# mdolab/dafoam

Hardware: AMD Instinct MI355X
Metric: adjoint_gmres_iterations_per_sec (higher is better)
Workload: dtype f64

## Files before the change

dafoam_amd/_capi.py:

```python
from __future__ import annotations

import ctypes as C
import os

import numpy as np

from .meshgen import FoamCase

_HERE = os.path.dirname(os.path.abspath(__file__))
LIB_PATH = os.environ.get("DAFOAM_AMD_LIB") or os.path.join(_HERE, "lib", "libdafoam_amd.so")

SOLVER_IDS = {"DASimpleFoam": 0, "DAScalarTransportFoam": 1, "DARhoSimpleFoam": 2, "DATurboFoam": 3}
PATCH_TYPES = {"patch": 0, "wall": 1, "symmetry": 2, "cyclic": 3}

c_double_p = C.POINTER(C.c_double)
c_int_p = C.POINTER(C.c_int)
c_ll_p = C.POINTER(C.c_longlong)


class das_case_t(C.Structure):
    _fields_ = [
        ("solver", C.c_int),
        ("n_points", C.c_int),
        ("n_faces", C.c_int),
# ... 238 lines not shown
    "das_set_dense_eig_callback": (C.c_int, [_VP]),
    "das_debug_gmres_dr_host": (C.c_int, [C.c_longlong, _VP, _VP, _VP, c_double_p, c_double_p, C.c_int, C.c_int, C.c_double, C.c_double, C.c_longlong, c_double_p, C.c_int,
                                          c_double_p, c_double_p]),
    "das_debug_gmres_dr_restart": (C.c_int, [C.c_int, C.c_int, c_double_p, c_double_p, c_double_p, c_double_p, c_double_p]),
    "das_ksp_get_status": (C.c_int, [_VP, c_int_p, c_int_p, c_int_p, c_int_p]),
    "das_ksp_get_pc_stability": (C.c_int, [_VP, C.POINTER(C.c_double), c_int_p]),
    "das_ksp_get_pc_subdomains": (C.c_int, [_VP, c_int_p, c_double_p]),
    "das_ksp_get_pc_node_out": (C.c_int, [_VP, c_int_p]),
    "das_mesh_metrics": (C.c_int, [C.c_int, c_double_p, C.c_int, C.c_int, C.c_int, c_int_p, c_int_p, c_int_p, c_int_p, c_double_p, c_double_p, c_double_p, c_double_p, c_double_p]),
    "das_ksp_get_coarse": (C.c_int, [_VP, c_int_p]),
    "das_ksp_coarse_sparse_az_active": (C.c_int, [_VP]),
    "das_ksp_set_global_coarse": (C.c_int, [_VP, _VP, C.c_int, C.c_int, c_int_p]),
    "das_ksp_run_fixed_device": (C.c_int, [_VP, _VP, _VP, _VP, C.c_int]),
    "das_ksp_begin_device": (C.c_int, [_VP, _VP, _VP, _VP, C.c_int]),
    "das_ksp_advance": (C.c_int, [_VP, _VP, C.c_int]),
    "das_ksp_end": (C.c_int, [_VP, _VP]),
    "das_ksp_destroy": (None, [_VP]),
    "das_set_owned_mask": (C.c_int, [_VP, C.POINTER(C.c_ubyte)]),
    "das_comm_load_rccl": (C.c_int, []),
    "das_comm_unique_id": (C.c_int, [C.c_char_p]),
    "das_comm_init_rccl": (C.c_int, [_VP, C.c_int, C.c_int, C.c_char_p]),
    "das_comm_set_halo": (C.c_int, [_VP, C.c_int, c_int_p, c_ll_p, c_int_p, c_ll_p, c_int_p, C.c_longlong, c_int_p]),
    "das_set_exchange_cb": (C.c_int, [_VP, _VP, _VP]),
    "das_set_pc_overlap": (C.c_int, [_VP, C.POINTER(C.c_ubyte), C.c_int, c_ll_p, c_int_p, c_ll_p, c_int_p]),
    "das_set_gather_cb": (C.c_int, [_VP, _VP, _VP]),
    "das_comm_is_native": (C.c_int, [_VP]),
    "das_comm_reset": (C.c_int, [_VP]),
    "das_set_comm": (C.c_int, [_VP, _VP, _VP, _VP]),
    "das_set_stream": (C.c_int, [_VP, _VP]),
    "das_get_elapsed_clock_time": (C.c_double, [_VP]),
    "das_get_elapsed_cpu_time": (C.c_double, [_VP]),
    "das_timer_avg_ms": (C.c_double, [_VP, C.c_char_p]),
    "das_debug_orth_bench": (C.c_int, [C.c_longlong, C.c_int, C.c_int, C.c_int, C.c_int, C.c_int, C.POINTER(C.c_double), C.POINTER(C.c_double)]),
    "das_debug_krylov_dots2": (C.c_int, [C.c_longlong, C.c_int, C.c_int, _VP, C.c_longlong, c_double_p, c_double_p]),
    "das_debug_krylov_dcgs2_update": (C.c_int, [C.c_longlong, C.c_int, C.c_int, _VP, C.c_longlong, C.c_int, c_double_p, C.c_double, C.c_double, c_double_p]),
    "das_debug_krylov_multidot": (C.c_int, [C.c_longlong, C.c_int, C.c_int, _VP, C.c_longlong, c_double_p, c_double_p]),
    "das_debug_krylov_multiaxpy": (C.c_int, [C.c_longlong, C.c_int, C.c_int, _VP, C.c_longlong, c_double_p, C.c_int, _VP, C.c_longlong]),
    "das_debug_krylov_lincomb": (C.c_int, [C.c_longlong, C.c_int, C.c_int, _VP, C.c_longlong, c_double_p, c_double_p, C.c_longlong]),
    "das_debug_krylov_scale_to": (C.c_int, [C.c_longlong, C.c_double, C.c_int, _VP, _VP, C.c_longlong]),
    "das_debug_krylov_block_tn": (C.c_int, [C.c_longlong, C.c_int, C.c_int, c_double_p, C.c_longlong, C.c_longlong, c_double_p, C.c_longlong, c_double_p]),
    "das_debug_krylov_block_nn_sub": (C.c_int, [C.c_longlong, C.c_int, C.c_int, c_double_p, C.c_longlong, c_double_p, c_double_p, C.c_longlong]),
    "das_debug_krylov_block_right_mult": (C.c_int, [C.c_longlong, C.c_int, c_double_p, C.c_longlong, c_double_p]),
    "das_debug_krylov_block_lincomb": (C.c_int, [C.c_longlong, C.c_int, C.c_int, c_double_p, C.c_longlong, c_double_p, c_double_p, C.c_longlong]),
    "das_debug_krylov_block_spmm": (C.c_int, [C.c_longlong, C.c_int, c_ll_p, c_int_p, c_double_p, c_double_p, C.c_longlong, c_double_p, C.c_longlong]),
    "das_timer_count": (C.c_longlong, [_VP, C.c_char_p]),
    "das_timer_reset": (None, [_VP]),
    "das_timer_enable": (None, [_VP, C.c_int]),
}

_lib = None


def declared_symbols():
    return sorted(_SIGS)


def lib():
    global _lib
    if _lib is None:
        if not os.path.exists(LIB_PATH):
            raise ImportError(
                f"{LIB_PATH} not found: build the HIP extension first (python -c 'import __graft_entry__ as g; g.build()'). "
                "dafoam_amd has no CPU fallback."
            )
        L = C.CDLL(LIB_PATH)
        for name, (res, args) in _SIGS.items():
# ... 45 lines not shown
```

dafoam_amd/csrc/das_device.hip:

```cpp
#include <algorithm>
#include <cmath>
#include <ctime>
#include <functional>
#include <numeric>
#include <thread>

#include "das_case.hpp"
#include "das_jaccon.hpp"
#include "das_bilu.hpp"
#include "das_comm.hpp"
#include "das_block.hpp"
#include "das_color.hpp"
#include "das_opmat.hpp"
#include "das_graph.hpp"
#include "das_volcoord.hpp"
#include "das_cellfn.hpp"
#include "das_simple.hpp"

#include <omp.h>

namespace das {

template <class T, bool RHO, class G = double>
__global__ __launch_bounds__(256) void k_grad(DevMeshT<G> m, ResParams prm, const T* __restrict__ W, T* nut, T* gU, T* gP, T* gN, T* gH) {
// ... 506 lines not shown
#pragma unroll
        for (int t = 0; t < UNROLL; t++)
#pragma unroll
            for (int r = 0; r < RPT; r++) q[t][r] = (double)V[(long long)(i + t) * ldv + kk[r]];
        if (Vlo) {
#pragma unroll
            for (int t = 0; t < UNROLL; t++)
#pragma unroll
                for (int r = 0; r < RPT; r++) q[t][r] += (double)Vlo[(long long)(i + t) * ldv + kk[r]];
        }
#pragma unroll
        for (int t = 0; t < UNROLL; t++)
#pragma unroll
            for (int r = 0; r < RPT; r++) { as[r] += s[i + t] * q[t][r]; ac[r] += c[i + t] * q[t][r]; }
    }
    for (; i < j; i++)
#pragma unroll
        for (int r = 0; r < RPT; r++) {
            const double q = (double)V[(long long)i * ldv + kk[r]] + (Vlo ? (double)Vlo[(long long)i * ldv + kk[r]] : 0.0);
            as[r] += s[i] * q; ac[r] += c[i] * q;
        }
#pragma unroll
    for (int r = 0; r < RPT; r++) {
        const long long k = k0 + (long long)r * blockDim.x;
        if (k >= n) continue;
        const double u = (double)V[(long long)j * ldv + k] + (Vlo ? (double)Vlo[(long long)j * ldv + k] : 0.0);
        const double qj = (u - as[r]) * ralpha, un = (v[k] - gamma * u - ac[r]) * ralpha;
        const VT qh = (VT)qj, uh = (VT)un;
        V[(long long)j * ldv + k] = qh;
        V[(long long)(j + 1) * ldv + k] = uh;
        if (Vlo) { Vlo[(long long)j * ldv + k] = (float)(qj - (double)qh); Vlo[(long long)(j + 1) * ldv + k] = (float)(un - (double)uh); }
    }
}
template <class VT>
__global__ __launch_bounds__(256) void k_lincomb(long long n, int m, const VT* __restrict__ V, long long ldv, const double* __restrict__ c,
                                                 double* __restrict__ y, const float* __restrict__ Vlo = nullptr) {
    long long k = (long long)blockIdx.x * blockDim.x + threadIdx.x;
    if (k >= n) return;
    double s = 0.0;
    if (Vlo) for (int i = 0; i < m; i++) s += c[i] * ((double)V[(long long)i * ldv + k] + (double)Vlo[(long long)i * ldv + k]);
    else for (int i = 0; i < m; i++) s += c[i] * (double)V[(long long)i * ldv + k];
    y[k] = s;
}
template <class TI, class TO>
__global__ void k_scale_to(long long n, double a, const TI* __restrict__ x, TO* __restrict__ y, const float* __restrict__ xlo = nullptr,
                           float* __restrict__ ylo = nullptr) {
    long long k = (long long)blockIdx.x * blockDim.x + threadIdx.x;
    if (k >= n) return;
    const double val = a * ((double)x[k] + (xlo ? (double)xlo[k] : 0.0));
    const TO yh = (TO)val;
    y[k] = yh;
    if (ylo) ylo[k] = (float)(val - (double)yh);
}
static inline size_t multidot_partial_size(long long n, int m) { return (size_t)(m + 1) * nblk(n, MD_CHUNK); }
template <class VT>
static void launch_multidot(hipStream_t st, long long n, int m, const VT* V, long long ldv, const double* w, double* partial, double* out) {
    const int nb = nblk(n, MD_CHUNK);
    hipLaunchKernelGGL(k_multidot, dim3(nb), dim3(256), 0, st, n, m, V, ldv, w, partial, nb);
    hipLaunchKernelGGL(k_reduce, dim3(m + 1), dim3(256), 0, st, nb, (const double*)partial, out);
}
template <int ROWS>
static inline long long multidot2_nbw(long long n) { return 4LL * nblk(n, 256 * ROWS); }
static inline size_t multidot2_partial_size(long long n, int K) { return (size_t)2 * K * (size_t)multidot2_nbw<MD2_ROWS>(n); }
template <int ROWS, class VT>
static void launch_multidot2_pass(hipStream_t st, long long n, int K, const VT* V, long long ldv, const VT* u, const double* v, double* partial) {
    hipLaunchKernelGGL((k_multidot2<ROWS, VT, VT>), dim3(nblk(n, 256 * ROWS)), dim3(256), 0, st, n, K, V, ldv, u, v, partial, multidot2_nbw<ROWS>(n));
}
template <class VT>
static void launch_multidot2(hipStream_t st, long long n, int K, const VT* V, long long ldv, const VT* u, const double* v, double* partial, double* out) {
    launch_multidot2_pass<MD2_ROWS, VT>(st, n, K, V, ldv, u, v, partial);
    hipLaunchKernelGGL(k_reduce, dim3(2 * K), dim3(256), 0, st, (int)multidot2_nbw<MD2_ROWS>(n), (const double*)partial, out);
}
template <int UNROLL, int RPT, class VT>
static void launch_dcgs2_update(hipStream_t st, long long n, int j, VT* V, long long ldv, const double* sc, double gamma, double ralpha, const double* v,
                                float* Vlo) {
    hipLaunchKernelGGL((k_dcgs2_update<UNROLL, RPT, VT>), dim3(nblk(n, 256 * RPT)), dim3(256), 0, st, n, j, V, ldv, sc, gamma, ralpha, v, Vlo);
}
template <class VT, class WT>
static void launch_multiaxpy(hipStream_t st, long long n, int m, const VT* V, long long ldv, const double* h, WT* w, const float* Vlo) {
    hipLaunchKernelGGL(k_multiaxpy, dim3(nblk(n, 256)), dim3(256), 0, st, n, m, V, ldv, h, w, Vlo);
}
template <class VT>
static void launch_lincomb(hipStream_t st, long long n, int m, const VT* V, long long ldv, const double* c, double* y, const float* Vlo) {
    hipLaunchKernelGGL(k_lincomb, dim3(nblk(n, 256)), dim3(256), 0, st, n, m, V, ldv, c, y, Vlo);
}
template <class TI, class TO>
static void launch_scale_to(hipStream_t st, long long n, double a, const TI* x, TO* y, const float* xlo, float* ylo) {
    hipLaunchKernelGGL(k_scale_to, dim3(nblk(n, 256)), dim3(256), 0, st, n, a, x, y, xlo, ylo);
}
static constexpr int TSG_CHUNKS = 1024;
static inline int tsgemm_kpad(int K) { return (K + 16 * TSG_TILES - 1) / (16 * TSG_TILES) * (16 * TSG_TILES); }
static inline size_t tsgemm_partial_size(int K) { return (size_t)TSG_CHUNKS * tsgemm_kpad(K) * 16; }
static void launch_tsgemm_tn(hipStream_t st, long long n, int K, int sv, const double* V, long long ldv, const double* W, long long ldw, double* partial,
                             double* C) {
    long long rpc = (n + TSG_CHUNKS - 1) / TSG_CHUNKS;
    rpc = (rpc + 15) / 16 * 16;
    const int Kpad = tsgemm_kpad(K);
    const int gy = Kpad / (16 * TSG_TILES);
    DAS_CHECK((((ldv | ldw) & 1) != 0) || ((((uintptr_t)V | (uintptr_t)W) & 15) == 0), DAS_ERR_ARG,
              "block V^T W: even leading dimensions need 16-byte aligned blocks");
    hipLaunchKernelGGL(k_tsgemm_tn, dim3(TSG_CHUNKS / TSG_WAVES, gy), dim3(64 * TSG_WAVES), 0, st, n, K, sv, V, ldv, W, ldw, rpc, Kpad, partial);
    hipLaunchKernelGGL(k_tsgemm_reduce, dim3(nblk((long long)K * sv, 4)), dim3(256), 0, st, K, sv, Kpad, (long long)TSG_CHUNKS, (const double*)partial, C);
}
static void launch_tsgemm_nn_sub(hipStream_t st, long long n, int K, int sv, const double* V, long long ldv, const double* C, double* W, long long ldw) {
    hipLaunchKernelGGL(k_tsgemm_nn_sub, dim3(nblk(n, 256)), dim3(256), 0, st, n, K, sv, V, ldv, C, W, ldw);
}
static void launch_block_right_mult(hipStream_t st, long long n, int sv, double* W, long long ldw, const double* T) {
    hipLaunchKernelGGL(k_block_right_mult, dim3(nblk(n, 256)), dim3(256), 0, st, n, sv, W, ldw, T);
// ... 1646 lines not shown
}

static void pc_apply(das_solver* s, das_ksp* k, const double* b, double* x) {
    hipEvent_t ev = nullptr;
    s->timer.begin("pc", s->stream, ev);
    if (k->useBilu) {
        if (k->rasOverlap) {
            DAS_HIP(hipMemcpyAsync(k->pcin.p, b, (size_t)s->n * sizeof(double), hipMemcpyDeviceToDevice, s->stream));
            s->halo.gather_overlap(k->pcin.p, s->stream);
            bilu_apply(k->bilu, k->pcin.p, x, s->stream);
            s->halo.zero_overlap(x, s->stream);
        } else {
            bilu_apply(k->bilu, b, x, s->stream);
        }
        s->timer.end("pc", s->stream, ev);
        return;
    }
    const int mlv = k->pc.maxLevels;
    const size_t lvlBytes = (size_t)((mlv + 2 * PC_PF + 4) >> 1) * sizeof(double);
    if (k->pc.useLDS)
        hipLaunchKernelGGL(k_ras_apply<true>, dim3(k->pc.nBlocks), dim3(PC_THREADS), lvlBytes + (size_t)k->pc.maxLocal * sizeof(double), s->stream,
                           k->pc.view, b, x, mlv);
    else
        hipLaunchKernelGGL(k_ras_apply<false>, dim3(k->pc.nBlocks), dim3(PC_THREADS), lvlBytes, s->stream, k->pc.view, b, x, mlv);
    s->timer.end("pc", s->stream, ev);
}

static void gmres_ws(das_solver* s, das_ksp* k) {
    const long long n = s->n;
    long long restart = std::min<long long>(s->opt.geti("adjEqnOption.gmresRestart"), s->opt.geti("adjEqnOption.gmresMaxIters"));
    long long budget = (long long)(32.0 * 1024 * 1024 * 1024);
    auto it = s->opt.i.find("amd.maxKrylovBytes");
    if (it != s->opt.i.end()) budget = it->second;
    const long long maxVec = std::max<long long>(3, budget / (8 * n));
    restart = std::max<long long>(1, std::min<long long>(restart, maxVec - 2));
    long long wantVec = std::max<long long>(restart + 2, std::min<long long>(maxVec, 1002));
    if ((size_t)wantVec * (size_t)n * sizeof(double) < ((size_t)4 << 30) || getenv("DAS_NO_VMM")) wantVec = restart + 2;
    if (k->V.n < (size_t)((restart + 2) * n) || k->Vn != n) {
        k->V.reserve((size_t)(wantVec * n));
        k->Vn = n;
    }
    {
        std::string prec = "auto";
        { auto ip = s->opt.s.find("amd.krylovBasisPrecision"); if (ip != s->opt.s.end()) prec = ip->second; }
        DAS_CHECK(prec == "auto" || prec == "fp64" || prec == "fp32" || prec == "split", DAS_ERR_ARG, "amd.krylovBasisPrecision: auto | fp64 | split | fp32");
        const bool eligible = s->opt.geti("adjEqnOption.useMGSO") == 0 && !s->fwd.on;
        const bool dcgs2 = s->opt.gets("amd.gmresOrthogonalization") == "dcgs2" && s->opt.geti("adjEqnOption.useMGSO") == 0;
        bool big = (size_t)(restart + 2) * (size_t)n * 8 >= ((size_t)1 << 30);
        if (s->halo.active || s->allreduce_cb) {
            DevBuf<double> f(1);
            const double fv = big ? 1.0 : 0.0;
            DAS_HIP(hipMemcpyAsync(f.p, &fv, sizeof(double), hipMemcpyHostToDevice, s->stream));
            if (!(s->halo.active && s->halo.allreduce(f.p, 1, s->stream)) && s->allreduce_cb) s->allreduce_cb(f.p, 1, s->comm_user);
            DAS_HIP(hipStreamSynchronize(s->stream));
            big = f.to_host()[0] > 0.5;
        }
        k->split = eligible && (prec == "split" || (prec == "auto" && dcgs2 && big));
        k->vf32 = k->split || (eligible && prec == "fp32");
        if (k->vf32 && k->ustage.n != (size_t)n) k->ustage.alloc(n);
    }
    if (k->restart != restart || k->w.n != (size_t)n) {
        k->restart = (int)restart;
        k->w.alloc(n); k->z.alloc(n); k->r.alloc(n); k->xdev.alloc(n); k->bdev.alloc(n);
        k->z.zero();
        k->partial.alloc(std::max<size_t>(multidot_partial_size(n, (int)restart + 1), multidot2_partial_size(n, (int)restart + 2)));
        k->hdev.alloc(4 * (restart + 3));
    }
}
static inline bool gmres_map_basis(das_solver* s, das_ksp* k, long long nvec) {
    const long long per = (k->vf32 && !k->split) ? (s->n + 1) / 2 : s->n;
    k->V.request((size_t)((nvec + 64) * per));
    return k->V.try_ensure((size_t)(nvec * per));
}
static inline long long basis_ld(das_solver* s, das_ksp* k) { return k->split ? 2 * s->n : s->n; }
template <class VT>
static inline VT* basis_slot(das_solver* s, das_ksp* k, long long j) { return reinterpret_cast<VT*>(k->V.p) + j * basis_ld(s, k); }
static inline float* basis_lo(das_solver* s, das_ksp* k, long long j) { return k->split ? reinterpret_cast<float*>(k->V.p) + j * basis_ld(s, k) + s->n : nullptr; }

template <class VT>
static void multidot_dev(das_solver* s, das_ksp* k, const VT* Vbase, int m, const double* w, double* dev_out) {
    launch_multidot<VT>(s->stream, s->n, m, Vbase, basis_ld(s, k), w, k->partial.p, dev_out);
    if (!(s->halo.active && s->halo.allreduce(dev_out, m + 1, s->stream)) && s->allreduce_cb) s->allreduce_cb(dev_out, m + 1, s->comm_user);
}
template <class VT = double>
static void multidot(das_solver* s, das_ksp* k, int m, const double* w, double* h_host) {
    multidot_dev<VT>(s, k, basis_slot<VT>(s, k, 0), m, w, k->hdev.p);
    DAS_HIP(hipMemcpyAsync(h_host, k->hdev.p, (m + 1) * sizeof(double), hipMemcpyDeviceToHost, s->stream));
    DAS_HIP(hipStreamSynchronize(s->stream));
}

static void apply_operator(das_solver* s, const double* x, double* y);

static bool coarse_az_ready(das_solver* s, das_ksp* k) {
    das_ksp::CoarsePC& C = k->coarse;
    if (!s->op || s->fwd.on) return false;
    { auto it = s->opt.i.find("amd.pcCoarseSparseAZ"); if (it != s->opt.i.end() && it->second == 0) return false; }
    const Mat& A = s->op->m;
    if (C.azOpId == s->opId && C.azEpoch == s->op_epoch) return C.azReady;
    C.azOpId = s->opId; C.azEpoch = s->op_epoch; C.azReady = false; C.azFailed = false;
    const long long n = s->n;
    hipStream_t st = s->stream;
    DevBuf<int> cnt(n), ovf(1);
    DAS_HIP(hipMemsetAsync(ovf.p, 0, sizeof(int), st));
    hipLaunchKernelGGL(k_az_build, dim3(nblk(n, 256)), dim3(256), 0, st, n, A.rowptr.p, A.col.p, A.val.p, C.N, C.off, C.agg.p, 0, cnt.p, (const long long*)nullptr,
                       (int*)nullptr, (double*)nullptr, ovf.p);
    DAS_HIP(hipStreamSynchronize(st));
    int ovfAny = ovf.to_host()[0];
    if (s->halo.active || s->allreduce_cb) {
        DevBuf<double> f(1);
        const double fv = ovfAny ? 1.0 : 0.0;
// ... 1077 lines not shown
            info.steps = step + 1;
            info.hist.push_back(rn);
            if (s->opt.geti("debug")) fprintf(stderr, "[dafoam_amd] Newton primal step %d: REJECTED (|R| would be %.3e, %d GMRES iterations), tau -> %.2e\n", step + 1, rnew, k->iters, tau);
            if (++nRejected > 40) break;
            continue;
        }
        DAS_HIP(hipMemcpyAsync(s->d_W.p, Wn.p, n * sizeof(double), hipMemcpyDeviceToDevice, st));
        DAS_HIP(hipMemcpyAsync(Rc.p, Rn.p, n * sizeof(double), hipMemcpyDeviceToDevice, st));
        const double tauNew = !ramp ? std::min(1e12, tau0 * std::pow(info.res0 / std::max(rnew, 1e-300), serExp))
                                    : std::min(tauMax, tau * (omega == 1.0 ? std::max(growth, std::min(growthMax, std::pow(rn / std::max(rnew, 1e-300), serExp))) : std::max(omega, 0.25)));
        if (tauNew > 4.0 * tauPC || tauNew < 0.25 * tauPC) sincePC = pcLag;
        tau = std::max(tauMin, tauNew);
        rn = rnew;
        info.steps = step + 1;
        info.hist.push_back(rn);
        if (s->opt.geti("debug")) fprintf(stderr, "[dafoam_amd] Newton primal step %d: |R| %.3e (omega %.3f, %d GMRES iterations, tau %.2e)\n", step + 1, rn, omega, k->iters, tau);
    }
    DAS_HIP(hipStreamSynchronize(st));
    s->h_W = s->d_W.to_host();
    info.res = rn;
    info.seconds = wall_seconds() - t0;
    return (rn <= std::max(relTol * info.res0, absTol)) ? 0 : 1;
}

template <int ROWS>
static void orth_bench_dots(long long n, int K, const double* V, const double* w, double* partial) {
    launch_multidot2_pass<ROWS, double>(0, n, K, V, n, V + (long long)(K - 1) * n, w, partial);
}
template <int UNROLL, int RPT>
static void orth_bench_update(long long n, int j, double* V, const double* sc, const double* w) {
    launch_dcgs2_update<UNROLL, RPT, double>(0, n, j, V, n, sc, 0.5, 1.0, w, (float*)nullptr);
}

enum { KRY_FP64 = 0, KRY_FP32 = 1, KRY_SPLIT = 2 };
static void krylov_check_basis(const std::string& who, long long n, long long nvec, int fmt, const void* V, long long ld) {
    DAS_CHECK(n > 0 && nvec > 0, DAS_ERR_ARG, who + ": sizes must be positive");
    DAS_CHECK(fmt == KRY_FP64 || fmt == KRY_FP32 || fmt == KRY_SPLIT, DAS_ERR_ARG, who + ": fmt is 0 (fp64), 1 (fp32) or 2 (split)");
    DAS_CHECK(V, DAS_ERR_ARG, who + ": null basis");
    DAS_CHECK(ld >= (fmt == KRY_SPLIT ? 2 * n : n), DAS_ERR_ARG, who + ": leading dimension below n (split: below 2 n)");
}
static void krylov_check_block(const std::string& who, long long n, int K, int sv) {
    DAS_CHECK(n > 0 && K > 0, DAS_ERR_ARG, who + ": sizes must be positive");
    DAS_CHECK(sv >= 1 && sv <= 8, DAS_ERR_ARG, who + ": 1 to 8 right-hand sides");
}
static void krylov_debug_sync() {
    DAS_HIP(hipGetLastError());
    DAS_HIP(hipStreamSynchronize(0));
}
template <class VT>
static float* krylov_lo(VT* V, long long n, bool split) { return split ? reinterpret_cast<float*>(V) + n : nullptr; }
template <class VT>
static void debug_krylov_dots2(long long n, int K, const void* V, long long ld, const double* v, double* out) {
    DevBuf<VT> dV;
    dV.upload((const VT*)V, (size_t)K * ld);
    DevBuf<double> dv, partial(multidot2_partial_size(n, K)), dout((size_t)2 * K);
    dv.upload(v, n);
    launch_multidot2<VT>(0, n, K, (const VT*)dV.p, ld, (const VT*)(dV.p + (long long)(K - 1) * ld), (const double*)dv.p, partial.p, dout.p);
    krylov_debug_sync();
    dout.download(out, (size_t)2 * K);
}
template <class VT>
static void debug_krylov_dcgs2_update(long long n, int j, bool split, void* V, long long ld, int nslots, const double* sc, double gamma, double ralpha,
                                      const double* v) {
    DevBuf<VT> dV;
    dV.upload((const VT*)V, (size_t)nslots * ld);
    DevBuf<double> dsc((size_t)std::max(1, 2 * j)), dv;
// ... 1863 lines not shown
    return k->coarse.nagg;
}
int das_ksp_set_global_coarse(das_solver_t* s, das_ksp_t* k, int naggGlobal, int aggOffset, const int* aggRowGlobal) {
    DAS_TRY
    need_init(s);
    DAS_CHECK(k && aggRowGlobal, DAS_ERR_ARG, "null argument");
    das_ksp::CoarsePC& C = k->coarse;
    DAS_CHECK(C.N > 0 && !C.h_agg.empty(), DAS_ERR_STATE, "the preconditioner of this KSP has no coarse space (amd.pcCoarseAggregates)");
    DAS_CHECK(aggOffset >= 0 && aggOffset + C.nagg <= naggGlobal, DAS_ERR_ARG, "aggregate offset out of range");
    std::vector<int> rows(aggRowGlobal, aggRowGlobal + C.N);
    for (long long c = 0; c < C.N; c++) {
        DAS_CHECK(rows[c] >= -1 && rows[c] < naggGlobal, DAS_ERR_ARG, "global aggregate id out of range");
        if (C.h_agg[c] >= 0) DAS_CHECK(rows[c] == aggOffset + C.h_agg[c], DAS_ERR_ARG, "owned cells must carry offset + local aggregate");
    }
    coarse_build_operator(s, k, naggGlobal, aggOffset, rows);
    if (C.active) return DAS_OK;
    coarse_build_operator(s, k, C.nagg, 0, C.h_agg);
    return 1;
    DAS_CATCH
}
int das_ksp_get_history(das_ksp_t* k, double* hist, int cap) {
    DAS_TRY
    DAS_CHECK(k && hist, DAS_ERR_ARG, "null argument");
    int m = std::min<int>(cap, (int)k->hist.size());
    std::copy(k->hist.begin(), k->hist.begin() + m, hist);
    return m;
    DAS_CATCH
}
int das_ksp_get_basis_info(das_ksp_t* k, int* fp32, double* mappedBytes, double* bytesPerVector) {
    DAS_TRY
    DAS_CHECK(k, DAS_ERR_ARG, "null argument");
    if (fp32) *fp32 = ((k->vf32 && !k->split) ? 1 : 0) | (k->split ? 2 : 0);
    if (mappedBytes) *mappedBytes = (double)k->V.mappedBytes;
    if (bytesPerVector) *bytesPerVector = (double)k->Vn * ((k->vf32 && !k->split) ? 4.0 : 8.0);
    return DAS_OK;
    DAS_CATCH
}
int das_ksp_get_cycle_lengths(das_ksp_t* k, int* lens, int cap) {
    DAS_TRY
    DAS_CHECK(k && (lens || cap == 0), DAS_ERR_ARG, "null argument");
    int m = std::min<int>(cap, (int)k->cycleLens.size());
    std::copy(k->cycleLens.begin(), k->cycleLens.begin() + m, lens);
    return (int)k->cycleLens.size();
    DAS_CATCH
}
int das_ksp_run_fixed_device(das_solver_t* s, das_ksp_t* ksp, const double* d_rhs, double* d_sol, int iters) {
    DAS_TRY
    DAS_CHECK(ksp && d_rhs && d_sol && iters > 0, DAS_ERR_ARG, "bad argument");
    return run_gmres(s, ksp, d_rhs, d_sol, iters);
    DAS_CATCH
}
int das_ksp_begin_device(das_solver_t* s, das_ksp_t* ksp, const double* d_rhs, double* d_sol, int fixed) {
    DAS_TRY
    DAS_CHECK(ksp && d_rhs && d_sol, DAS_ERR_ARG, "bad argument");
    gmres_begin(s, ksp, d_rhs, d_sol, fixed != 0);
    return DAS_OK;
    DAS_CATCH
}
int das_ksp_advance(das_solver_t* s, das_ksp_t* ksp, int iters) {
    DAS_TRY
    DAS_CHECK(ksp && ksp->run && iters > 0, DAS_ERR_STATE, "das_ksp_begin_device has not been called");
    return gmres_advance(s, ksp, iters) ? 1 : 0;
    DAS_CATCH
}
int das_ksp_end(das_solver_t* s, das_ksp_t* ksp) {
    DAS_TRY
    DAS_CHECK(ksp && ksp->run, DAS_ERR_STATE, "das_ksp_begin_device has not been called");
// ... 133 lines not shown
    DAS_CATCH
}

int das_debug_orth_bench(long long n, int K, int reps, int rows, int unroll, int rpt, double* ms_dots, double* ms_update) {
    DAS_TRY
    DAS_CHECK(n > 0 && K > 1 && reps > 0 && ms_dots && ms_update, DAS_ERR_ARG, "das_debug_orth_bench: bad arguments");
    DevBuf<double> V((size_t)(K + 2) * n), w(n), partial((size_t)2 * K * 4 * nblk(n, 256 * 4)), sc(2 * (size_t)K);
    V.zero(); w.zero(); sc.zero();
    hipEvent_t e0, e1;
    DAS_HIP(hipEventCreate(&e0)); DAS_HIP(hipEventCreate(&e1));
    auto timed = [&](auto&& launch) {
        launch();
        DAS_HIP(hipEventRecord(e0, 0));
        for (int r = 0; r < reps; r++) launch();
        DAS_HIP(hipEventRecord(e1, 0));
        DAS_HIP(hipEventSynchronize(e1));
        DAS_HIP(hipGetLastError());
        float ms = 0.f;
        DAS_HIP(hipEventElapsedTime(&ms, e0, e1));
        return (double)ms / reps;
    };
    *ms_dots = -1.0; *ms_update = -1.0;
    if (rows == 4) *ms_dots = timed([&] { orth_bench_dots<4>(n, K, V.p, w.p, partial.p); });
    else if (rows == 8) *ms_dots = timed([&] { orth_bench_dots<8>(n, K, V.p, w.p, partial.p); });
    else if (rows == 16) *ms_dots = timed([&] { orth_bench_dots<16>(n, K, V.p, w.p, partial.p); });
#define DAS_UPD(U, R) if (unroll == U && rpt == R) *ms_update = timed([&] { orth_bench_update<U, R>(n, K - 1, V.p, sc.p, w.p); })
    DAS_UPD(4, 1); DAS_UPD(8, 1); DAS_UPD(16, 1); DAS_UPD(4, 2); DAS_UPD(8, 2); DAS_UPD(4, 4); DAS_UPD(8, 4);
#undef DAS_UPD
    (void)hipEventDestroy(e0); (void)hipEventDestroy(e1);
    return DAS_OK;
    DAS_CATCH
}

int das_debug_krylov_dots2(long long n, int K, int fmt, const void* V, long long ld, const double* v, double* out) {
    DAS_TRY
    krylov_check_basis("das_debug_krylov_dots2", n, K, fmt, V, ld);
    DAS_CHECK(v && out, DAS_ERR_ARG, "das_debug_krylov_dots2: null pointer");
    if (fmt == KRY_FP64) debug_krylov_dots2<double>(n, K, V, ld, v, out);
    else debug_krylov_dots2<float>(n, K, V, ld, v, out);
    return DAS_OK;
    DAS_CATCH
}
int das_debug_krylov_dcgs2_update(long long n, int j, int fmt, void* V, long long ld, int nslots, const double* sc, double gamma, double ralpha,
                                  const double* v) {
    DAS_TRY
    DAS_CHECK(j >= 0, DAS_ERR_ARG, "das_debug_krylov_dcgs2_update: j must not be negative");
    krylov_check_basis("das_debug_krylov_dcgs2_update", n, nslots, fmt, V, ld);
    DAS_CHECK(nslots >= j + 2, DAS_ERR_ARG, "das_debug_krylov_dcgs2_update: the basis needs slots 0 .. j + 1");
    DAS_CHECK(v && (sc || j == 0), DAS_ERR_ARG, "das_debug_krylov_dcgs2_update: null pointer");
    if (fmt == KRY_FP64) debug_krylov_dcgs2_update<double>(n, j, false, V, ld, nslots, sc, gamma, ralpha, v);
    else debug_krylov_dcgs2_update<float>(n, j, fmt == KRY_SPLIT, V, ld, nslots, sc, gamma, ralpha, v);
    return DAS_OK;
    DAS_CATCH
}
int das_debug_krylov_multidot(long long n, int m, int fmt, const void* V, long long ld, const double* w, double* out) {
    DAS_TRY
    DAS_CHECK(m >= 0, DAS_ERR_ARG, "das_debug_krylov_multidot: m must not be negative");
    krylov_check_basis("das_debug_krylov_multidot", n, std::max(m, 1), fmt, m > 0 ? V : (const void*)w, ld);
    DAS_CHECK(w && out, DAS_ERR_ARG, "das_debug_krylov_multidot: null pointer");
    if (fmt == KRY_FP64) debug_krylov_multidot<double>(n, m, V, ld, w, out);
    else debug_krylov_multidot<float>(n, m, V, ld, w, out);
    return DAS_OK;
    DAS_CATCH
}
int das_debug_krylov_multiaxpy(long long n, int m, int fmt, const void* V, long long ld, const double* h, int wfloat, void* w, long long wlen) {
    DAS_TRY
// ... 142 lines not shown
```

include/dafoam_amd.h:

```cpp
#ifndef DAFOAM_AMD_H
#define DAFOAM_AMD_H

#ifdef __cplusplus
extern "C" {
#endif

#define DAS_OK 0
#define DAS_ERR_ARG -1
#define DAS_ERR_NO_DEVICE -2
#define DAS_ERR_HIP -3
#define DAS_ERR_STATE -4
#define DAS_ERR_INTERNAL -5

#define DAS_SOLVER_SIMPLEFOAM 0
#define DAS_SOLVER_SCALARTRANSPORTFOAM 1
#define DAS_SOLVER_RHOSIMPLEFOAM 2
#define DAS_SOLVER_TURBOFOAM 3
#define DAS_IS_COMPRESSIBLE(s) ((s) == DAS_SOLVER_RHOSIMPLEFOAM || (s) == DAS_SOLVER_TURBOFOAM)

#define DAS_PATCH_PATCH 0
#define DAS_PATCH_WALL 1
#define DAS_PATCH_SYMMETRY 2
#define DAS_PATCH_CYCLIC 3

// ... 167 lines not shown
int das_ksp_get_pc_stability(das_ksp_t* ksp, double* estimate, int* orderUsed);
int das_ksp_get_pc_subdomains(das_ksp_t* ksp, int* orders, double* estimates);
int das_ksp_get_coarse(das_ksp_t* ksp, int* aggOfCell);
int das_ksp_coarse_sparse_az_active(das_ksp_t* ksp);
int das_ksp_set_global_coarse(das_solver_t* s, das_ksp_t* ksp, int naggGlobal, int aggOffset, const int* aggRowGlobal);
int das_ksp_run_fixed_device(das_solver_t* s, das_ksp_t* ksp, const double* d_rhs, double* d_sol, int iters);
int das_ksp_begin_device(das_solver_t* s, das_ksp_t* ksp, const double* d_rhs, double* d_sol, int fixed);
int das_ksp_advance(das_solver_t* s, das_ksp_t* ksp, int iters);
int das_ksp_end(das_solver_t* s, das_ksp_t* ksp);
void das_ksp_destroy(das_ksp_t* k);

typedef void (*das_halo_cb)(double* d_vec, void* user);
typedef void (*das_allreduce_cb)(double* d_buf, int n, void* user);
int das_set_owned_mask(das_solver_t* s, const unsigned char* owned );
int das_set_comm(das_solver_t* s, das_halo_cb halo, das_allreduce_cb allreduce, void* user);
int das_comm_load_rccl(void);
typedef void (*das_exchange_cb)(double* d_send, double* d_recv, void* user);
int das_comm_unique_id(char* out128);
int das_comm_init_rccl(das_solver_t* s, int rank, int world, const char* id128);
int das_comm_set_halo(das_solver_t* s, int npeers, const int* peers, const long long* sendOff, const int* sendIdx, const long long* recvOff,
                      const int* recvIdx, long long nGhost, const int* ghostIdx);
int das_set_exchange_cb(das_solver_t* s, das_exchange_cb cb, void* user);
int das_set_pc_overlap(das_solver_t* s, const unsigned char* pcMask , int npeers, const long long* ovSendOff, const int* ovSendIdx,
                       const long long* ovRecvOff, const int* ovRecvIdx);
int das_set_gather_cb(das_solver_t* s, das_exchange_cb cb, void* user);
int das_comm_is_native(das_solver_t* s);
int das_comm_reset(das_solver_t* s);
int das_set_stream(das_solver_t* s, void* hip_stream);

double das_get_elapsed_clock_time(das_solver_t* s);
double das_get_elapsed_cpu_time(das_solver_t* s);
double das_timer_avg_ms(das_solver_t* s, const char* name);
int das_debug_orth_bench(long long n, int K, int reps, int rows, int unroll, int rpt, double* ms_dots, double* ms_update);
int das_debug_krylov_dots2(long long n, int K, int fmt, const void* V, long long ld, const double* v, double* out);
int das_debug_krylov_dcgs2_update(long long n, int j, int fmt, void* V, long long ld, int nslots, const double* sc, double gamma, double ralpha,
                                  const double* v);
int das_debug_krylov_multidot(long long n, int m, int fmt, const void* V, long long ld, const double* w, double* out);
int das_debug_krylov_multiaxpy(long long n, int m, int fmt, const void* V, long long ld, const double* h, int wfloat, void* w, long long wlen);
int das_debug_krylov_lincomb(long long n, int m, int fmt, const void* V, long long ld, const double* c, double* y, long long ylen);
int das_debug_krylov_scale_to(long long n, double a, int use, const void* x, void* y, long long ylen);
int das_debug_krylov_block_tn(long long n, int K, int s, const double* V, long long ldv, long long voff, const double* W, long long ldw, double* C);
int das_debug_krylov_block_nn_sub(long long n, int K, int s, const double* V, long long ldv, const double* C, double* W, long long ldw);
int das_debug_krylov_block_right_mult(long long n, int s, double* W, long long ldw, const double* T);
int das_debug_krylov_block_lincomb(long long n, int K, int s, const double* V, long long ldv, const double* C, double* Y, long long ldy);
int das_debug_krylov_block_spmm(long long n, int s, const long long* rowptr, const int* colidx, const double* vals, const double* X, long long ldx,
                                double* Y, long long ldy);
long long das_timer_count(das_solver_t* s, const char* name);
void das_timer_reset(das_solver_t* s);
void das_timer_enable(das_solver_t* s, int on);

#ifdef __cplusplus
}
#endif
#endif
```

Before: 41.18.

## Add 128-bit vectorized fp32 Krylov orthogonalization kernels with padded basis layout

Adds wide multidot2 and DCGS2 update kernels for fp32 and split-fp32 Krylov bases. Each thread loads four floats as one 128-bit vector, optionally with nontemporal loads, and the kernels use a multi-level shuffle reduction. The basis leading dimension is padded to a multiple of four so the vector loads stay aligned. This targets the memory bandwidth of the orthogonalization in GMRES. It costs more code paths and extra padding memory, and the kernel falls back to the old path when alignment checks fail.

```diff
diff --git a/dafoam_amd/_capi.py b/dafoam_amd/_capi.py
--- a/dafoam_amd/_capi.py
+++ b/dafoam_amd/_capi.py
@@ -294,6 +294,9 @@
     "das_get_elapsed_cpu_time": (C.c_double, [_VP]),
     "das_timer_avg_ms": (C.c_double, [_VP, C.c_char_p]),
     "das_debug_orth_bench": (C.c_int, [C.c_longlong, C.c_int, C.c_int, C.c_int, C.c_int, C.c_int, C.POINTER(C.c_double), C.POINTER(C.c_double)]),
+    "das_debug_orth_bench_split": (C.c_int, [C.c_longlong, C.c_int, C.c_int, C.c_int, C.c_int, C.c_int, C.c_int, C.c_int, C.POINTER(C.c_double), C.POINTER(C.c_double)]),
+    "das_debug_set_orth_wide": (C.c_int, [C.c_int, C.POINTER(C.c_int)]),
+    "das_debug_krylov_wide_eligible": (C.c_int, [C.c_longlong, C.c_int, C.c_longlong, C.POINTER(C.c_int), C.POINTER(C.c_int)]),
     "das_debug_krylov_dots2": (C.c_int, [C.c_longlong, C.c_int, C.c_int, _VP, C.c_longlong, c_double_p, c_double_p]),
     "das_debug_krylov_dcgs2_update": (C.c_int, [C.c_longlong, C.c_int, C.c_int, _VP, C.c_longlong, C.c_int, c_double_p, C.c_double, C.c_double, c_double_p]),
     "das_debug_krylov_multidot": (C.c_int, [C.c_longlong, C.c_int, C.c_int, _VP, C.c_longlong, c_double_p, c_double_p]),
diff --git a/dafoam_amd/csrc/das_device.hip b/dafoam_amd/csrc/das_device.hip
--- a/dafoam_amd/csrc/das_device.hip
+++ b/dafoam_amd/csrc/das_device.hip
@@ -562,6 +562,202 @@
         if (Vlo) { Vlo[(long long)j * ldv + k] = (float)(qj - (double)qh); Vlo[(long long)(j + 1) * ldv + k] = (float)(un - (double)uh); }
     }
 }
+typedef float f32x4 __attribute__((ext_vector_type(4)));
+typedef double f64x2 __attribute__((ext_vector_type(2)));
+template <bool FULL, bool NT>
+__device__ __forceinline__ f32x4 ld_group(const float* __restrict__ vec, const unsigned (&bo)[4]) {
+    const char* b = reinterpret_cast<const char*>(vec);
+    if (FULL) {
+        const f32x4* p = reinterpret_cast<const f32x4*>(b + bo[0]);
+        return NT ? __builtin_nontemporal_load(p) : *p;
+    }
+    f32x4 r;
+    r.x = *reinterpret_cast<const float*>(b + bo[0]);
+    r.y = *reinterpret_cast<const float*>(b + bo[1]);
+    r.z = *reinterpret_cast<const float*>(b + bo[2]);
+    r.w = *reinterpret_cast<const float*>(b + bo[3]);
+    return r;
+}
+template <bool FULL>
+__device__ __forceinline__ void group_offsets(long long k, long long n, unsigned (&bo)[4]) {
+#pragma unroll
+    for (int e = 0; e < 4; e++) bo[e] = (unsigned)((FULL ? k + e : min(k + e, n - 1)) * 4);
+}
+template <int R4, bool FULL, bool NT>
+__device__ __forceinline__ void multidot2w_body(long long n, int K, const float* __restrict__ V, long long ldv, const float* __restrict__ u,
+                                                const double* __restrict__ v, double* __restrict__ partial, long long nbw) {
+    const int lane = threadIdx.x & 63, g = lane >> 3;
+    const long long base = ((long long)blockIdx.x * (256 * R4) + threadIdx.x) * 4;
+    const long long slot = (long long)blockIdx.x * 4 + (threadIdx.x >> 6);
+    unsigned bo[R4][4];
+    float ur[R4][4];
+    double vr[R4][4];
+#pragma unroll
+    for (int t = 0; t < R4; t++) {
+        const long long k = base + 1024LL * t;
+        group_offsets<FULL>(k, n, bo[t]);
+        const f32x4 uu = ld_group<FULL, false>(u, bo[t]);
+        ur[t][0] = uu.x; ur[t][1] = uu.y; ur[t][2] = uu.z; ur[t][3] = uu.w;
+        if (FULL) {
+            const f64x2 a = *reinterpret_cast<const f64x2*>(v + k), b = *reinterpret_cast<const f64x2*>(v + k + 2);
+            vr[t][0] = a.x; vr[t][1] = a.y; vr[t][2] = b.x; vr[t][3] = b.y;
+        } else {
+#pragma unroll
+            for (int e = 0; e < 4; e++) {
+                const bool in = k + e < n;
+                vr[t][e] = in ? v[min(k + e, n - 1)] : 0.0;
+                ur[t][e] = in ? ur[t][e] : 0.f;
+            }
+        }
+    }
+    const float* v0 = V;
+    for (int i0 = 0; i0 < K; i0 += 4, v0 += 4 * ldv) {
+        f32x4 x[4][R4];
+        double acc[8];
+#pragma unroll
+        for (int ii = 0; ii < 4; ii++) {
+            const float* vi = v0 + (long long)min(ii, K - 1 - i0) * ldv;
+#pragma unroll
+            for (int t = 0; t < R4; t++) x[ii][t] = ld_group<FULL, NT>(vi, bo[t]);
+        }
+#pragma unroll
+        for (int ii = 0; ii < 4; ii++) {
+            double a = 0.0, b = 0.0;
+#pragma unroll
+            for (int t = 0; t < R4; t++) {
+                const double x0 = (double)x[ii][t].x, x1 = (double)x[ii][t].y, x2 = (double)x[ii][t].z, x3 = (double)x[ii][t].w;
+                a += x0 * (double)ur[t][0]; b += x0 * vr[t][0];
+                a += x1 * (double)ur[t][1]; b += x1 * vr[t][1];
+                a += x2 * (double)ur[t][2]; b += x2 * vr[t][2];
+                a += x3 * (double)ur[t][3]; b += x3 * vr[t][3];
+            }
+            acc[2 * ii] = a;
+            acc[2 * ii + 1] = b;
+        }
+        double a4[4], a2[2], a1;
+#pragma unroll
+        for (int i = 0; i < 4; i++) {
+            const double snd = (g & 4) ? acc[i] : acc[i + 4], keep = (g & 4) ? acc[i + 4] : acc[i];
+            a4[i] = keep + __shfl_xor(snd, 32, 64);
+        }
+#pragma unroll
+        for (int i = 0; i < 2; i++) {
+            const double snd = (g & 2) ? a4[i] : a4[i + 2], keep = (g & 2) ? a4[i + 2] : a4[i];
+            a2[i] = keep + __shfl_xor(snd, 16, 64);
+        }
+        {
+            const double snd = (g & 1) ? a2[0] : a2[1], keep = (g & 1) ? a2[1] : a2[0];
+            a1 = keep + __shfl_xor(snd, 8, 64);
+        }
+        a1 += __shfl_xor(a1, 1, 64);
+        a1 += __shfl_xor(a1, 2, 64);
+        a1 += __shfl_xor(a1, 4, 64);
+        const int i = i0 + (g >> 1);
+        if ((lane & 7) == 0 && i < K) partial[((long long)(g & 1) * K + i) * nbw + slot] = a1;
+    }
+}
+template <int R4, bool NT>
+__global__ __launch_bounds__(256) void k_multidot2w(long long n, int K, const float* __restrict__ V, long long ldv, const float* __restrict__ u,
+                                                    const double* __restrict__ v, double* __restrict__ partial, long long nbw) {
+    if ((long long)(blockIdx.x + 1) * (1024 * R4) <= n) multidot2w_body<R4, true, NT>(n, K, V, ldv, u, v, partial, nbw);
+    else multidot2w_body<R4, false, NT>(n, K, V, ldv, u, v, partial, nbw);
+}
+template <int UNROLL, int RPT4, bool FULL, bool NT>
+__device__ __forceinline__ void dcgs2w_body(long long n, int j, float* __restrict__ V, long long ldv, const double* __restrict__ sc, double gamma,
+                                            double ralpha, const double* __restrict__ v, float* __restrict__ Vlo) {
+    const long long base = ((long long)blockIdx.x * (256 * RPT4) + threadIdx.x) * 4;
+    const double* s = sc;
+    const double* c = sc + j;
+    unsigned bo[RPT4][4];
+    double as[RPT4][4], ac[RPT4][4];
+#pragma unroll
+    for (int r = 0; r < RPT4; r++) {
+        group_offsets<FULL>(base + 1024LL * r, n, bo[r]);
+#pragma unroll
+        for (int e = 0; e < 4; e++) { as[r][e] = 0.0; ac[r][e] = 0.0; }
+    }
+    const float* h0 = V;
+    const float* l0 = Vlo;
+    for (int i = 0; i < j; i += UNROLL, h0 += UNROLL * ldv, l0 += (Vlo ? UNROLL * ldv : 0)) {
+        f32x4 qh[UNROLL][RPT4], ql[UNROLL][RPT4];
+#pragma unroll
+        for (int t = 0; t < UNROLL; t++) {
+            const float* hv = h0 + (long long)min(t, j - 1 - i) * ldv;
+#pragma unroll
+            for (int r = 0; r < RPT4; r++) qh[t][r] = ld_group<FULL, NT>(hv, bo[r]);
+        }
+        if (Vlo) {
+#pragma unroll
+            for (int t = 0; t < UNROLL; t++) {
+                const float* lv = l0 + (long long)min(t, j - 1 - i) * ldv;
+#pragma unroll
+                for (int r = 0; r < RPT4; r++) ql[t][r] = ld_group<FULL, NT>(lv, bo[r]);
+            }
+        }
+#pragma unroll
+        for (int t = 0; t < UNROLL; t++) {
+            const bool in = i + t < j;
+            const double st = in ? s[min(i + t, j - 1)] : 0.0, ct = in ? c[min(i + t, j - 1)] : 0.0;
+#pragma unroll
+            for (int r = 0; r < RPT4; r++) {
+                double q[4] = {(double)qh[t][r].x, (double)qh[t][r].y, (double)qh[t][r].z, (double)qh[t][r].w};
+                if (Vlo) { q[0] += (double)ql[t][r].x; q[1] += (double)ql[t][r].y; q[2] += (double)ql[t][r].z; q[3] += (double)ql[t][r].w; }
+#pragma unroll
+                for (int e = 0; e < 4; e++) { as[r][e] += st * q[e]; ac[r][e] += ct * q[e]; }
+            }
+        }
+    }
+    float* uh = V + (long long)j * ldv;
+    float* nh = uh + ldv;
+    float* ul = Vlo ? Vlo + (long long)j * ldv : nullptr;
+    float* nl = Vlo ? ul + ldv : nullptr;
+#pragma unroll
+    for (int r = 0; r < RPT4; r++) {
+        const long long k = base + 1024LL * r;
+        if (k >= n) continue;
+        const f32x4 u4 = ld_group<FULL, false>(uh, bo[r]);
+        double u[4] = {(double)u4.x, (double)u4.y, (double)u4.z, (double)u4.w}, vv[4];
+        if (Vlo) {
+            const f32x4 l4 = ld_group<FULL, false>(ul, bo[r]);
+            u[0] += (double)l4.x; u[1] += (double)l4.y; u[2] += (double)l4.z; u[3] += (double)l4.w;
+        }
+        if (FULL) {
+            const f64x2 a = *reinterpret_cast<const f64x2*>(v + k), b = *reinterpret_cast<const f64x2*>(v + k + 2);
+            vv[0] = a.x; vv[1] = a.y; vv[2] = b.x; vv[3] = b.y;
+        } else {
+#pragma unroll
+            for (int e = 0; e < 4; e++) vv[e] = v[min(k + e, n - 1)];
+        }
+        float qh[4], qlo[4], nhh[4], nlo[4];
+#pragma unroll
+        for (int e = 0; e < 4; e++) {
+            const double qj = (u[e] - as[r][e]) * ralpha, un = (vv[e] - gamma * u[e] - ac[r][e]) * ralpha;
+            qh[e] = (float)qj; nhh[e] = (float)un;
+            qlo[e] = (float)(qj - (double)qh[e]); nlo[e] = (float)(un - (double)nhh[e]);
+        }
+        if (FULL) {
+            *reinterpret_cast<f32x4*>(uh + k) = f32x4{qh[0], qh[1], qh[2], qh[3]};
+            *reinterpret_cast<f32x4*>(nh + k) = f32x4{nhh[0], nhh[1], nhh[2], nhh[3]};
+            if (Vlo) {
+                *reinterpret_cast<f32x4*>(ul + k) = f32x4{qlo[0], qlo[1], qlo[2], qlo[3]};
+                *reinterpret_cast<f32x4*>(nl + k) = f32x4{nlo[0], nlo[1], nlo[2], nlo[3]};
+            }
+        } else {
+#pragma unroll
+            for (int e = 0; e < 4; e++) {
+                if (k + e >= n) continue;
+                uh[k + e] = qh[e]; nh[k + e] = nhh[e];
+                if (Vlo) { ul[k + e] = qlo[e]; nl[k + e] = nlo[e]; }
+            }
+        }
+    }
+}
+template <int UNROLL, int RPT4, bool NT>
+__global__ __launch_bounds__(256) void k_dcgs2w_update(long long n, int j, float* __restrict__ V, long long ldv, const double* __restrict__ sc,
+                                                       double gamma, double ralpha, const double* __restrict__ v, float* __restrict__ Vlo) {
+    if ((long long)(blockIdx.x + 1) * (1024 * RPT4) <= n) dcgs2w_body<UNROLL, RPT4, true, NT>(n, j, V, ldv, sc, gamma, ralpha, v, Vlo);
+    else dcgs2w_body<UNROLL, RPT4, false, NT>(n, j, V, ldv, sc, gamma, ralpha, v, Vlo);
+}
 template <class VT>
 __global__ __launch_bounds__(256) void k_lincomb(long long n, int m, const VT* __restrict__ V, long long ldv, const double* __restrict__ c,
                                                  double* __restrict__ y, const float* __restrict__ Vlo = nullptr) {
@@ -591,19 +787,66 @@
 }
 template <int ROWS>
 static inline long long multidot2_nbw(long long n) { return 4LL * nblk(n, 256 * ROWS); }
-static inline size_t multidot2_partial_size(long long n, int K) { return (size_t)2 * K * (size_t)multidot2_nbw<MD2_ROWS>(n); }
+#ifndef MD2W_R4
+#define MD2W_R4 4
+#endif
+#ifndef MD2W_NT
+#define MD2W_NT 1
+#endif
+#ifndef DCGS2W_UNROLL
+#define DCGS2W_UNROLL 4
+#endif
+#ifndef DCGS2W_RPT4
+#define DCGS2W_RPT4 2
+#endif
+#ifndef DCGS2W_NT
+#define DCGS2W_NT 0
+#endif
+#ifndef ORTH_WIDE_DEFAULT
+#define ORTH_WIDE_DEFAULT 1
+#endif
+static int g_orth_wide = ORTH_WIDE_DEFAULT;
+static inline bool orth_wide_ok(long long n, const void* V, const void* Vlo, long long ldv, const void* u, const void* v) {
+    return n >= 4 && n < (1LL << 30) && (ldv & 3) == 0 && ((((uintptr_t)V | (uintptr_t)Vlo | (uintptr_t)u | (uintptr_t)v) & 15) == 0);
+}
+static inline long long multidot2w_nbw(long long n, int r4) { return 4LL * nblk(n, 1024 * r4); }
+static inline size_t multidot2_partial_size(long long n, int K) {
+    return (size_t)2 * K * (size_t)std::max(multidot2_nbw<MD2_ROWS>(n), multidot2w_nbw(n, MD2W_R4));
+}
 template <int ROWS, class VT>
 static void launch_multidot2_pass(hipStream_t st, long long n, int K, const VT* V, long long ldv, const VT* u, const double* v, double* partial) {
     hipLaunchKernelGGL((k_multidot2<ROWS, VT, VT>), dim3(nblk(n, 256 * ROWS)), dim3(256), 0, st, n, K, V, ldv, u, v, partial, multidot2_nbw<ROWS>(n));
 }
+template <int R4, bool NT>
+static void launch_multidot2w_pass(hipStream_t st, long long n, int K, const float* V, long long ldv, const float* u, const double* v, double* partial) {
+    hipLaunchKernelGGL((k_multidot2w<R4, NT>), dim3(nblk(n, 1024 * R4)), dim3(256), 0, st, n, K, V, ldv, u, v, partial, multidot2w_nbw(n, R4));
+}
+template <int UNROLL, int RPT4, bool NT>
+static void launch_dcgs2w_update(hipStream_t st, long long n, int j, float* V, long long ldv, const double* sc, double gamma, double ralpha,
+                                 const double* v, float* Vlo) {
+    hipLaunchKernelGGL((k_dcgs2w_update<UNROLL, RPT4, NT>), dim3(nblk(n, 1024 * RPT4)), dim3(256), 0, st, n, j, V, ldv, sc, gamma, ralpha, v, Vlo);
+}
 template <class VT>
 static void launch_multidot2(hipStream_t st, long long n, int K, const VT* V, long long ldv, const VT* u, const double* v, double* partial, double* out) {
+    if constexpr (std::is_same<VT, float>::value) {
+        if (g_orth_wide && orth_wide_ok(n, V, nullptr, ldv, u, v)) {
+            launch_multidot2w_pass<MD2W_R4, MD2W_NT != 0>(st, n, K, V, ldv, u, v, partial);
+            hipLaunchKernelGGL(k_reduce, dim3(2 * K), dim3(256), 0, st, (int)multidot2w_nbw(n, MD2W_R4), (const double*)partial, out);
+            return;
+        }
+    }
     launch_multidot2_pass<MD2_ROWS, VT>(st, n, K, V, ldv, u, v, partial);
     hipLaunchKernelGGL(k_reduce, dim3(2 * K), dim3(256), 0, st, (int)multidot2_nbw<MD2_ROWS>(n), (const double*)partial, out);
 }
 template <int UNROLL, int RPT, class VT>
 static void launch_dcgs2_update(hipStream_t st, long long n, int j, VT* V, long long ldv, const double* sc, double gamma, double ralpha, const double* v,
                                 float* Vlo) {
+    if constexpr (std::is_same<VT, float>::value) {
+        if (g_orth_wide && orth_wide_ok(n, V, Vlo, ldv, nullptr, v)) {
+            launch_dcgs2w_update<DCGS2W_UNROLL, DCGS2W_RPT4, DCGS2W_NT != 0>(st, n, j, V, ldv, sc, gamma, ralpha, v, Vlo);
+            return;
+        }
+    }
     hipLaunchKernelGGL((k_dcgs2_update<UNROLL, RPT, VT>), dim3(nblk(n, 256 * RPT)), dim3(256), 0, st, n, j, V, ldv, sc, gamma, ralpha, v, Vlo);
 }
 template <class VT, class WT>
@@ -2316,12 +2559,13 @@
     long long budget = (long long)(32.0 * 1024 * 1024 * 1024);
     auto it = s->opt.i.find("amd.maxKrylovBytes");
     if (it != s->opt.i.end()) budget = it->second;
-    const long long maxVec = std::max<long long>(3, budget / (8 * n));
+    const long long nr = (n + 3) / 4 * 4;
+    const long long maxVec = std::max<long long>(3, budget / (8 * nr));
     restart = std::max<long long>(1, std::min<long long>(restart, maxVec - 2));
     long long wantVec = std::max<long long>(restart + 2, std::min<long long>(maxVec, 1002));
-    if ((size_t)wantVec * (size_t)n * sizeof(double) < ((size_t)4 << 30) || getenv("DAS_NO_VMM")) wantVec = restart + 2;
-    if (k->V.n < (size_t)((restart + 2) * n) || k->Vn != n) {
-        k->V.reserve((size_t)(wantVec * n));
+    if ((size_t)wantVec * (size_t)nr * sizeof(double) < ((size_t)4 << 30) || getenv("DAS_NO_VMM")) wantVec = restart + 2;
+    if (k->V.n < (size_t)((restart + 2) * nr) || k->Vn != n) {
+        k->V.reserve((size_t)(wantVec * nr));
         k->Vn = n;
     }
     {
@@ -2351,15 +2595,16 @@
         k->hdev.alloc(4 * (restart + 3));
     }
 }
+static inline long long basis_n4(das_solver* s) { return (s->n + 3) / 4 * 4; }
+static inline long long basis_ld(das_solver* s, das_ksp* k) { return k->split ? 2 * basis_n4(s) : (k->vf32 ? basis_n4(s) : s->n); }
 static inline bool gmres_map_basis(das_solver* s, das_ksp* k, long long nvec) {
-    const long long per = (k->vf32 && !k->split) ? (s->n + 1) / 2 : s->n;
+    const long long per = basis_ld(s, k) / (k->vf32 ? 2 : 1);
     k->V.request((size_t)((nvec + 64) * per));
     return k->V.try_ensure((size_t)(nvec * per));
 }
-static inline long long basis_ld(das_solver* s, das_ksp* k) { return k->split ? 2 * s->n : s->n; }
 template <class VT>
 static inline VT* basis_slot(das_solver* s, das_ksp* k, long long j) { return reinterpret_cast<VT*>(k->V.p) + j * basis_ld(s, k); }
-static inline float* basis_lo(das_solver* s, das_ksp* k, long long j) { return k->split ? reinterpret_cast<float*>(k->V.p) + j * basis_ld(s, k) + s->n : nullptr; }
+static inline float* basis_lo(das_solver* s, das_ksp* k, long long j) { return k->split ? reinterpret_cast<float*>(k->V.p) + j * basis_ld(s, k) + basis_n4(s) : nullptr; }
 
 template <class VT>
 static void multidot_dev(das_solver* s, das_ksp* k, const VT* Vbase, int m, const double* w, double* dev_out) {
@@ -3503,6 +3748,23 @@
     launch_dcgs2_update<UNROLL, RPT, double>(0, n, j, V, n, sc, 0.5, 1.0, w, (float*)nullptr);
 }
 
+template <int ROWS>
+static void orth_bench_dots_f(long long n, int K, const float* V, long long ld, const double* w, double* partial) {
+    launch_multidot2_pass<ROWS, float>(0, n, K, V, ld, V + (long long)(K - 1) * ld, w, partial);
+}
+template <int UNROLL, int RPT>
+static void orth_bench_update_f(long long n, int j, float* V, long long ld, float* lo, const double* sc, const double* w) {
+    hipLaunchKernelGGL((k_dcgs2_update<UNROLL, RPT, float>), dim3(nblk(n, 256 * RPT)), dim3(256), 0, 0, n, j, V, ld, sc, 0.5, 1.0, w, lo);
+}
+template <int R4, bool NT>
+static void orth_bench_dots_w(long long n, int K, const float* V, long long ld, const double* w, double* partial) {
+    launch_multidot2w_pass<R4, NT>(0, n, K, V, ld, V + (long long)(K - 1) * ld, w, partial);
+}
+template <int UNROLL, int RPT4, bool NT>
+static void orth_bench_update_w(long long n, int j, float* V, long long ld, float* lo, const double* sc, const double* w) {
+    launch_dcgs2w_update<UNROLL, RPT4, NT>(0, n, j, V, ld, sc, 0.5, 1.0, w, lo);
+}
+
 enum { KRY_FP64 = 0, KRY_FP32 = 1, KRY_SPLIT = 2 };
 static void krylov_check_basis(const std::string& who, long long n, long long nvec, int fmt, const void* V, long long ld) {
     DAS_CHECK(n > 0 && nvec > 0, DAS_ERR_ARG, who + ": sizes must be positive");
@@ -5432,7 +5694,7 @@
     DAS_CHECK(k, DAS_ERR_ARG, "null argument");
     if (fp32) *fp32 = ((k->vf32 && !k->split) ? 1 : 0) | (k->split ? 2 : 0);
     if (mappedBytes) *mappedBytes = (double)k->V.mappedBytes;
-    if (bytesPerVector) *bytesPerVector = (double)k->Vn * ((k->vf32 && !k->split) ? 4.0 : 8.0);
+    if (bytesPerVector) *bytesPerVector = k->vf32 ? (double)((k->Vn + 3) / 4 * 4) * (k->split ? 8.0 : 4.0) : (double)k->Vn * 8.0;
     return DAS_OK;
     DAS_CATCH
 }
@@ -5632,6 +5894,61 @@
     DAS_CATCH
 }
 
+int das_debug_orth_bench_split(long long n, int K, int reps, int fmt, int variant, int rows, int unroll, int rpt, double* ms_dots, double* ms_update) {
+    DAS_TRY
+    DAS_CHECK(n > 0 && n < (1LL << 30) && K > 1 && reps > 0 && ms_dots && ms_update, DAS_ERR_ARG, "das_debug_orth_bench_split: bad arguments");
+    DAS_CHECK((fmt == KRY_FP32 || fmt == KRY_SPLIT) && variant >= 0 && variant <= 2, DAS_ERR_ARG, "das_debug_orth_bench_split: fmt 1 | 2, variant 0 | 1 | 2");
+    const long long n4 = (n + 3) / 4 * 4, ld = fmt == KRY_SPLIT ? 2 * n4 : n4;
+    DevBuf<float> V((size_t)(K + 2) * ld);
+    DevBuf<double> w(n4), partial((size_t)2 * K * 4 * nblk(n, 1024)), sc(2 * (size_t)K);
+    V.zero(); w.zero(); sc.zero();
+    float* lo = fmt == KRY_SPLIT ? V.p + n4 : nullptr;
+    hipEvent_t e0, e1;
+    DAS_HIP(hipEventCreate(&e0)); DAS_HIP(hipEventCreate(&e1));
+    auto timed = [&](auto&& launch) {
+        launch();
+        DAS_HIP(hipEventRecord(e0, 0));
+        for (int r = 0; r < reps; r++) launch();
+        DAS_HIP(hipEventRecord(e1, 0));
+        DAS_HIP(hipEventSynchronize(e1));
+        DAS_HIP(hipGetLastError());
+        float ms = 0.f;
+        DAS_HIP(hipEventElapsedTime(&ms, e0, e1));
+        return (double)ms / reps;
+    };
+    *ms_dots = -1.0; *ms_update = -1.0;
+    const int j = K - 1;
+#define DAS_DOT(R) if (rows == R) *ms_dots = timed([&] { orth_bench_dots_f<R>(n, K, V.p, ld, w.p, partial.p); })
+#define DAS_UPD(U, R) if (unroll == U && rpt == R) *ms_update = timed([&] { orth_bench_update_f<U, R>(n, j, V.p, ld, lo, sc.p, w.p); })
+    if (variant == 0) { DAS_DOT(4); DAS_DOT(8); DAS_DOT(16); DAS_UPD(4, 1); DAS_UPD(8, 1); DAS_UPD(4, 2); DAS_UPD(8, 2); DAS_UPD(4, 4); }
+#undef DAS_DOT
+#undef DAS_UPD
+#define DAS_DOT(R, NT) if (rows == R) *ms_dots = timed([&] { orth_bench_dots_w<R, NT>(n, K, V.p, ld, w.p, partial.p); })
+#define DAS_UPD(U, R, NT) if (unroll == U && rpt == R) *ms_update = timed([&] { orth_bench_update_w<U, R, NT>(n, j, V.p, ld, lo, sc.p, w.p); })
+    if (variant == 1) { DAS_DOT(1, false); DAS_DOT(2, false); DAS_DOT(4, false); DAS_UPD(2, 1, false); DAS_UPD(4, 1, false); DAS_UPD(8, 1, false); DAS_UPD(2, 2, false); DAS_UPD(4, 2, false); }
+    if (variant == 2) { DAS_DOT(1, true); DAS_DOT(2, true); DAS_DOT(4, true); DAS_UPD(2, 1, true); DAS_UPD(4, 1, true); DAS_UPD(8, 1, true); DAS_UPD(2, 2, true); DAS_UPD(4, 2, true); }
+#undef DAS_DOT
+#undef DAS_UPD
+    (void)hipEventDestroy(e0); (void)hipEventDestroy(e1);
+    return DAS_OK;
+    DAS_CATCH
+}
+int das_debug_set_orth_wide(int on, int* previous) {
+    if (previous) *previous = g_orth_wide;
+    g_orth_wide = on ? 1 : 0;
+    return DAS_OK;
+}
+int das_debug_krylov_wide_eligible(long long n, int fmt, long long ld, int* dots, int* update) {
+    DAS_TRY
+    DAS_CHECK(dots && update, DAS_ERR_ARG, "das_debug_krylov_wide_eligible: null pointer");
+    const float* base = reinterpret_cast<const float*>((uintptr_t)1 << 20);
+    const bool f = fmt == KRY_FP32 || fmt == KRY_SPLIT;
+    *dots = (f && g_orth_wide && orth_wide_ok(n, base, nullptr, ld, base + ld, base)) ? 1 : 0;
+    *update = (f && g_orth_wide && orth_wide_ok(n, base, fmt == KRY_SPLIT ? base + n : nullptr, ld, nullptr, base)) ? 1 : 0;
+    return DAS_OK;
+    DAS_CATCH
+}
+
 int das_debug_krylov_dots2(long long n, int K, int fmt, const void* V, long long ld, const double* v, double* out) {
     DAS_TRY
     krylov_check_basis("das_debug_krylov_dots2", n, K, fmt, V, ld);
diff --git a/include/dafoam_amd.h b/include/dafoam_amd.h
--- a/include/dafoam_amd.h
+++ b/include/dafoam_amd.h
@@ -223,6 +223,9 @@
 double das_get_elapsed_cpu_time(das_solver_t* s);
 double das_timer_avg_ms(das_solver_t* s, const char* name);
 int das_debug_orth_bench(long long n, int K, int reps, int rows, int unroll, int rpt, double* ms_dots, double* ms_update);
+int das_debug_orth_bench_split(long long n, int K, int reps, int fmt, int variant, int rows, int unroll, int rpt, double* ms_dots, double* ms_update);
+int das_debug_set_orth_wide(int on, int* previous);
+int das_debug_krylov_wide_eligible(long long n, int fmt, long long ld, int* dots, int* update);
 int das_debug_krylov_dots2(long long n, int K, int fmt, const void* V, long long ld, const double* v, double* out);
 int das_debug_krylov_dcgs2_update(long long n, int j, int fmt, void* V, long long ld, int nslots, const double* sc, double gamma, double ralpha,
                                   const double* v);
```

Result: faster. 43.67 (median of 6 runs) (+6.0%).
